# Arktis2022/Spiking-Diffusion

Hardware: AMD Instinct MI355X
Metric: images/sec + LIF-kernel HBM GB/s, MNIST 100-step sample T=16, 1->8 GPU (higher is better)
Workload: dtype fp32-exact (4 fp6 digits x fp4 spikes on the block-scaled MFMA + certified decisions + exact 6-digit recomputation of flagged neurons)

## Files before the change

spiking-diffusion_amd/csrc/den_mfma_fp6v2.hip:

```cpp
#include "den_common.h"
#include "../../include/spkdiff.h"
#include <math.h>
#include <stdlib.h>
#include <type_traits>
#include <utility>

namespace {

typedef int v6i __attribute__((ext_vector_type(6)));
typedef int v8i __attribute__((ext_vector_type(8)));
typedef float v16f __attribute__((ext_vector_type(16)));

constexpr int T16 = 16;
constexpr int CK = 32;
constexpr int POSB = T16 * CK / 2;
constexpr int WT = 64 * 24;
constexpr int N_PAIR = 18;
constexpr int N_D4 = 5;
constexpr int N_MAIN = N_PAIR + N_D4;
constexpr int N_L5 = 2;
constexpr int NACC = 2;
constexpr int W_PIECES = (N_PAIR * WT + 1023) / 1024;
constexpr int W_LDS = W_PIECES * 1024;
constexpr int W_SLAB = ((N_MAIN + N_L5) * WT + 1023) / 1024 * 1024;

constexpr unsigned FLAG_CAP = 1u << 20;

struct V2Args {
  const uint8_t* in0; int nch;
  const uint8_t* wq; const double* scale; const double* bias; const float* wl1;
  const float* bn_a; const float* bn_b;
  uint8_t* out; uint8_t* out_cnt;
  unsigned* flags;
  unsigned flag_cap;
  long long ticket_idx;
  int handover;
  const int* qtab;
  const int* n_dyn;
  const uint8_t* need; const int* cls_cnt; const int* cls_list;
  int B, Cout, Cin;
  int gx, nsets;
};

#define SPK_FP6_PRE "s_nop 1\n\t"
#define SPK_MFMA2(CLS, acc, av, bv, sa, sb)                                                                          \
  asm volatile(SPK_FP6_PRE "v_mfma_scale_f32_32x32x64_f8f6f4 %0, %1, %2, %0, %3, %4 op_sel_hi:[0,0,0] cbsz:4 blgp:2"  \
               : "+" CLS(acc) : "v"(av), "v"(bv), "v"(sa), "v"(sb))
#define SPK_MFMA2_Z(CLS, acc, av, bv, sa, sb)                                                                        \
  asm volatile(SPK_FP6_PRE "v_mfma_scale_f32_32x32x64_f8f6f4 %0, %1, %2, 0, %3, %4 op_sel_hi:[0,0,0] cbsz:4 blgp:2"   \
               : "=&" CLS(acc) : "v"(av), "v"(bv), "v"(sa), "v"(sb))

constexpr int SPK_V2_KMIN = 2;
constexpr float SPK_V2_SPARE = 1.0f;
constexpr int SPK_V2_REC_STEP = 13;
constexpr int SPK_V2_LP_PAIRS = 1;
constexpr int SPK_V2_GX_KB = 2560;
constexpr int SPK_V2_HALF_FILL = 2;
constexpr int SPK_V2_LPS_MIN_B = 64;
constexpr int SPK_V2_LP_SPLIT_MAX = 512;
constexpr int SPK_V2_PF = 6;

constexpr float CERT_4EPS = 4.0f * 2.38418579e-07f;

__device__ __forceinline__ void store_tile_spikes(uint8_t* out, uint8_t* out_cnt, unsigned mybits, int lane, long long rec_base,
                                                  long long cnt_base, bool ok) {
  const unsigned bitsv = spk_transpose16_rows(mybits, lane);
  if (out_cnt && ok) out_cnt[cnt_base + (lane & 31)] = (uint8_t)__popc(mybits);
  if (ok) *reinterpret_cast<uint2*>(out + rec_base + (lane & 15) * 16 + 8 * ((lane >> 4) & 1)) = spk_e2m1_record(bitsv);
}

__device__ const uint8_t V2_HALF_REC[2][64] = {
    {0, 1, 2, 3, 4, 5, 6, 7, 8, 9, 10, 11, 12, 13, 14, 15, 16, 17, 18, 19, 20, 21, 22, 23,
     23, 23, 23, 23, 23, 23, 23, 23, 23, 23, 23, 23, 23, 23, 23, 23, 23, 23, 23, 23, 23, 23, 23, 23, 24},
    {24, 25, 26, 27, 28, 29, 30, 31, 32, 33, 34, 35, 36, 37, 38, 39, 40, 41, 42, 43, 44, 45, 46, 47,
     47, 47, 47, 47, 47, 47, 47, 47, 47, 47, 47, 47, 47, 47, 47, 47, 47, 47, 47, 47, 47, 47, 47, 47, 24}};

template <int H, int W, int NWV, bool SPLIT, int NTP, bool HALF = false>
__device__ __forceinline__ void fp6v2_body(const V2Args& a, const int g, const int il, const int lanes, const int n_images,
                                           const int* __restrict__ slots) {
  constexpr bool PRUNE = NTP > 0;
  static_assert(!HALF || (PRUNE && !SPLIT && H == 7 && W == 7 && NWV == 4 && NTP == 3), "half-image items: 7x7, four waves x three tiles");
  constexpr bool REC = !PRUNE;
  constexpr int HW = H * W, PW = W + 1;
  constexpr int Hb = SPLIT ? H / 2 : H;
  constexpr int Hin = SPLIT ? Hb + 1 : H;
  constexpr int HWb = Hb * W;
  static_assert(SPLIT ? ((H % 2) == 0 && (HWb % (2 * NWV)) == 0)
                      : ((HW & 1) == 1 && ((HW / 2) % NWV) == 0), "whole 32-row tiles on every wave (+ one odd position)");
  static_assert(!PRUNE || (!SPLIT && (NWV == 4 || NWV == 8) && NTP <= (HWb / 2) / NWV), "position lists: 7x7 items");
  constexpr int NT = PRUNE ? NTP : (HWb / 2) / NWV;
  constexpr int N_AGPR = NWV == 4 ? (NACC * NT < 16 ? NACC * NT : 16) : 0;
  constexpr int NPP = (Hin + 2) * PW + 1;
  constexpr int A_BYTES = NPP * POSB;
  constexpr int PPR = (W + 3) / 4;
  constexpr int NA = Hin * PPR;
  constexpr int NPA = (NA + NWV - 1) / NWV;
  constexpr int NPW = (W_PIECES + NWV - 1) / NWV;
  constexpr int NSTEP = 9 * NT;
  static_assert(NWV >= 8 || NACC * NT <= 16 || (NT - 1) * NACC <= N_AGPR + 2, "only the last tile may straddle the register files");
  constexpr bool AH = NWV == 8 && !PRUNE;
  constexpr int NBUF = 2;
  extern __shared__ __attribute__((aligned(16))) uint8_t lds[];
  uint8_t* const sA = lds;
  uint8_t* const sW = lds + NBUF * A_BYTES;
  int* const s_cin = reinterpret_cast<int*>(lds + NBUF * A_BYTES + NBUF * W_LDS);
  int* const s_row = s_cin + NPP * 16;
  int* const s_nmax = s_row + (HWb + 1) * 16;
  const unsigned sA_addr = spk_lds_addr(sA), sW_addr = sA_addr + NBUF * A_BYTES;
  const int tid = threadIdx.x, lane = tid & 63, wave = tid >> 6;
  const int nch = a.nch;
  const int G = a.Cout >> 5;
  for (int i = tid; i < NBUF * A_BYTES / 16; i += NWV * 64) reinterpret_cast<uint4*>(sA)[i] = make_uint4(0, 0, 0, 0);
  if (REC)
    for (int i = tid; i < NPP * 16; i += NWV * 64) s_cin[i] = 0;
  __syncthreads();

  const int row = lane & 31, half = lane >> 5;
  const int hsel = (row >> 2) & 1, tt = (row & 3) + 4 * (row >> 3);
  int a_off[NT];
  int p_out[NT];
#pragma unroll
  for (int i = 0; i < NT; ++i) {
    const int p = 2 * (wave + NWV * i) + hsel;
    a_off[i] = ((p / W) * PW + (p % W)) * POSB + tt * 16;
    p_out[i] = 2 * (wave + NWV * i) + half;
  }

  const int wave_s = __builtin_amdgcn_readfirstlane(wave);
  unsigned pa_pk[NPA];
#pragma unroll
  for (int j = 0; j < NPA; ++j) {
    int id = wave_s * NPA + j;
    id = id < NA ? id : NA - 1;
    const int y = id / PPR, px = id - y * PPR;
    const int np = (W - 4 * px) < 4 ? (W - 4 * px) : 4;
    const unsigned src = (unsigned)((y * W + 4 * px) * POSB), dst = (unsigned)(((y + 1) * PW + 1 + 4 * px) * POSB);
    pa_pk[j] = src | (dst << 14) | ((unsigned)(np - 1) << 29);
  }
  const unsigned lane16 = (unsigned)lane * 16u;
  const unsigned wave_k = (unsigned)wave_s * 1024u;
  auto issue_piece = [&](int q, const uint8_t* aslab, const uint8_t* wslab, unsigned dA, unsigned dW) {
    if (q < NPA) {
      const unsigned pk = pa_pk[q];
      const unsigned np = ((pk >> 29) & 3u) + 1u;
      const unsigned long long mask = np == 4 ? ~0ull : ((1ull << (16 * np)) - 1ull);
      spk_dma16s_masked(aslab + (pk & 0x3fffu), lane16, dA + ((pk >> 14) & 0x7fffu), mask);
    } else {
      unsigned ko = wave_k + 1024u * NWV * (unsigned)(q - NPA);
      if (NWV * (q - NPA) + NWV - 1 >= W_PIECES) ko = ko < (unsigned)W_PIECES * 1024u ? ko : ko - 1024u * NWV;
      spk_dma16s(wslab + ko, lane16, dW + ko);
    }
  };
  const uint8_t* const wbase = a.wq + (long long)g * nch * W_SLAB;
  auto aslab_of = [&](int itm, int c) -> const uint8_t* {
    const int b = HALF ? itm >> 1 : (PRUNE ? slots[itm] : (SPLIT ? itm >> 1 : itm)), band = SPLIT ? itm & 1 : 0;
    return a.in0 + ((long long)b * nch + c) * HW * POSB + band * (Hb - 1) * W * POSB;
  };
  const int nitems = (SPLIT || HALF) ? 2 * n_images : n_images;

  const int co = g * 32 + (lane & 31);
  const float scale_f = (float)a.scale[co], bias_f = (float)a.bias[co];
  const float bna = a.bn_a[co], bnb = a.bn_b[co];
  const float Bc = fmaf(bias_f, bna, bnb);
  const float cE = 2.0f * 2.38418579e-07f * (fabsf(bnb) + fabsf(Bc)) + 1e-30f;
  const float cT = 528.0f * scale_f * fabsf(bna) * 1.000001f;
  const float Ac4 = 1024.0f * scale_f * bna;

  const int sc_a = 0x7f7f7f7f;
  const int sc_p = half ? (int)0x82828282u : (int)0x87878787u;

  int it = 0;
  if (il < nitems) {
    const uint8_t* as0 = aslab_of(il, 0);
#pragma unroll
    for (int q = 0; q < NPA + NPW; ++q) issue_piece(q, as0, wbase, sA_addr, sW_addr);
    if constexpr (AH) {
      spk_dma_wait_all();
      __syncthreads();
    }
  }
  for (int itm = il; itm < nitems; itm += lanes) {
    const int b = HALF ? itm >> 1 : (PRUNE ? slots[itm] : (SPLIT ? itm >> 1 : itm)), band = SPLIT ? itm & 1 : 0;
    const int band_off = band * PW * POSB;
    int n_list = 2 * NT * NWV;
    if constexpr (PRUNE) {
      const uint8_t* rec = HALF ? &V2_HALF_REC[itm & 1][0] : a.need + (long long)b * 64;
      n_list = __builtin_amdgcn_readfirstlane((int)rec[48]);
#pragma unroll
      for (int i = 0; i < NT; ++i) {
        const int k2 = 2 * (wave + NWV * i);
        const int p = rec[k2 + hsel];
        a_off[i] = ((p / W) * PW + (p % W)) * POSB + tt * 16;
        p_out[i] = rec[k2 + half];
      }
    }
    v16f acc[NT][NACC];
    int cnt[NT];
#pragma unroll
    for (int i = 0; i < NT; ++i) cnt[i] = 0;
    constexpr int NREC = Hin * W * 16, NR = (NREC + NWV * 64 - 1) / (NWV * 64);
    int creg[NR];
    int rec_off[NR];
    bool rec_ok[NR];
#pragma unroll
    for (int k = 0; k < NR; ++k) {
      creg[k] = 0;
      const int r = tid + k * NWV * 64;
      const int cl = r >> 4, t = r & 15;
      rec_ok[k] = r < NREC;
      rec_off[k] = rec_ok[k] ? (((cl / W) + 1) * PW + 1 + (cl % W)) * POSB + t * 16 : 0;
    }
    constexpr int PFX = NWV == 4 ? SPK_V2_PF : 4;
    v6i bp[2][2];
    v4i af[PFX];
    for (int c = 0; c < nch; ++c, ++it) {
      const int buf = it & 1, buf1 = buf ^ 1;
      if constexpr (!AH) {
        spk_dma_wait_all();
        __syncthreads();
      }
      int nb = itm, nc = c + 1;
      if (nc == nch) { nc = 0; nb = itm + lanes; }
      const bool have_next = nb < nitems;
      const uint8_t* n_aslab = aslab_of(have_next ? nb : itm, have_next ? nc : c);
      const uint8_t* n_wslab = wbase + (long long)(have_next ? nc : c) * W_SLAB;
      const unsigned n_dA = sA_addr + buf1 * A_BYTES;
      const unsigned n_dW = sW_addr + buf1 * W_LDS;

      v4i rvq[NR];
      auto compute = [&](auto first_tag) {
        constexpr bool FIRST = decltype(first_tag)::value;
        const uint8_t* A = sA + buf * A_BYTES + band_off;
        const uint8_t* Wb = sW + buf * W_LDS;
        auto toff = [](int tap) constexpr -> int { return ((tap / 3) * PW + (tap % 3)) * POSB; };
        constexpr int NBLK = 9;
        auto lda = [&](auto s_tag) -> v4i {
          constexpr int s = decltype(s_tag)::value;
          constexpr int blk = s / NT, i = s % NT;
          return *reinterpret_cast<const v4i*>(A + a_off[i] + toff(blk));
        };
        auto ldb = [&](int tile) -> v6i {
          const uint8_t* p = Wb + tile * WT;
          const v4i x = *reinterpret_cast<const v4i*>(p + lane * 16);
          typedef const volatile __attribute__((address_space(3))) v2i* lds_v2i_ptr;
          const v2i y = *(lds_v2i_ptr)SPK_LDS(p + 1024 + lane * 8);
          const v6i r = {x[0], x[1], x[2], x[3], y[0], y[1]};
          return r;
        };
        constexpr int PF = PFX;
        if constexpr (!AH || FIRST) {
          bp[0][0] = ldb(0); bp[0][1] = ldb(1);
          static_for<PF>([&](auto s_tag) { af[decltype(s_tag)::value] = lda(s_tag); });
        }
        const uint8_t* An = sA + buf1 * A_BYTES + band_off;
        const uint8_t* Wn = sW + buf1 * W_LDS;
        const bool ahead = AH && c + 1 < nch;
        static_for<NSTEP>([&](auto s_tag) {
          constexpr int s = decltype(s_tag)::value;
          constexpr int blk = s / NT, i = s % NT;
          if constexpr (AH && s == NSTEP - PF) {
            asm volatile("s_waitcnt vmcnt(0)\n\ts_barrier" ::: "memory");
          }
          const v4i av = af[s % PF];
          if constexpr (s + PF < NSTEP) af[s % PF] = lda(std::integral_constant<int, s + PF>{});
          else if constexpr (AH) {
            constexpr int k = s % PF;
            if (ahead) af[k] = *reinterpret_cast<const v4i*>(An + a_off[k % NT] + toff(k / NT));
          }
          constexpr int NPIECES = NPA + NPW;
#define V2_DMA_SLOT()                                                                              \
  do {                                                                                             \
    if constexpr (i == 0 && 2 * blk < NPIECES) issue_piece(2 * blk, n_aslab, n_wslab, n_dA, n_dW);     \
    if constexpr (i == (NT > 1 ? NT / 2 : 0) && 2 * blk + 1 < NPIECES)                             \
      issue_piece(2 * blk + 1, n_aslab, n_wslab, n_dA, n_dW);                                      \
  } while (0)
#define V2_NEXT_TILES()                                                                            \
  do {                                                                                             \
    if constexpr (i == 0 && blk + 1 < NBLK) {                                                      \
      bp[(blk + 1) & 1][0] = ldb(2 * (blk + 1));                                                   \
      bp[(blk + 1) & 1][1] = ldb(2 * (blk + 1) + 1);                                               \
    }                                                                                              \
  } while (0)
          constexpr int tap = blk;
          if constexpr (!REC) {
            asm volatile("v_bcnt_u32_b32 %0, %1, %0\n\tv_bcnt_u32_b32 %0, %2, %0\n\tv_bcnt_u32_b32 %0, %3, %0\n\t"
                         "v_bcnt_u32_b32 %0, %4, %0" : "+v"(cnt[i]) : "v"(av[0]), "v"(av[1]), "v"(av[2]), "v"(av[3]));
          }
#define V2_PAIR_MFMA(J)                                                                                      \
do {                                                                                                        \
  if constexpr (FIRST && tap == 0) {                                                                        \
    if constexpr (NACC * i + (J) < N_AGPR) SPK_MFMA2_Z("a", acc[i][J], av, bp[0][J], sc_a, sc_p);              \
    else SPK_MFMA2_Z("v", acc[i][J], av, bp[0][J], sc_a, sc_p);                                             \
  } else {                                                                                                  \
    if constexpr (NACC * i + (J) < N_AGPR) SPK_MFMA2("a", acc[i][J], av, bp[tap & 1][J], sc_a, sc_p);          \
    else SPK_MFMA2("v", acc[i][J], av, bp[tap & 1][J], sc_a, sc_p);                                         \
  }                                                                                                         \
} while (0)
          V2_PAIR_MFMA(0);
          __builtin_amdgcn_sched_barrier(0);
          V2_DMA_SLOT();
          V2_NEXT_TILES();
          if constexpr (REC) {
            if constexpr (s == 1) {
#pragma unroll
              for (int k = 0; k < NR; ++k) rvq[k] = *reinterpret_cast<const v4i*>(sA + buf * A_BYTES + rec_off[k]);
            }
            if constexpr (s == SPK_V2_REC_STEP) {
#pragma unroll
              for (int k = 0; k < NR; ++k)
                creg[k] += __builtin_popcount((unsigned)rvq[k][0]) + __builtin_popcount((unsigned)rvq[k][1]) +
                           __builtin_popcount((unsigned)rvq[k][2]) + __builtin_popcount((unsigned)rvq[k][3]);
            }
          }
          V2_PAIR_MFMA(1);
          __builtin_amdgcn_sched_barrier(0);
          if constexpr (AH && s == NSTEP - 1) {
            if (ahead) {
              auto ldb_n = [&](int tile) -> v6i {
                const uint8_t* p = Wn + tile * WT;
                const v4i x = *reinterpret_cast<const v4i*>(p + lane * 16);
                typedef const volatile __attribute__((address_space(3))) v2i* lds_v2i_ptr;
                const v2i y = *(lds_v2i_ptr)SPK_LDS(p + 1024 + lane * 8);
                const v6i r = {x[0], x[1], x[2], x[3], y[0], y[1]};
                return r;
              };
              bp[0][0] = ldb_n(0); bp[0][1] = ldb_n(1);
            }
          }
        });
      };
      if (c == 0) compute(std::true_type{}); else compute(std::false_type{});
    }

    if constexpr (REC) {
#pragma unroll
      for (int k = 0; k < NR; ++k)
        if (rec_ok[k]) s_cin[(rec_off[k] / POSB) * 16 + ((rec_off[k] % POSB) >> 4)] = creg[k];
      if (tid <= HWb) s_nmax[tid] = 0;
      __syncthreads();
      for (int e = tid; e < HWb * 16; e += NWV * 64) {
        const int pp = e >> 4, t = e & 15;
        const int* c0 = s_cin + (((pp / W) + band) * PW + (pp % W)) * 16 + t;
        int sum = 0;
#pragma unroll
        for (int dy = 0; dy < 3; ++dy)
#pragma unroll
          for (int dx = 0; dx < 3; ++dx) sum += c0[(dy * PW + dx) * 16];
        s_row[e] = sum;
        atomicMax(&s_nmax[pp], sum);
      }
      __syncthreads();
    }
    asm volatile("s_nop 15\n\ts_nop 15" ::: "memory");

#pragma unroll
    for (int k = 0; k < NT; ++k) {
      const int i = k == 0 ? NT - 1 : k - 1;
#pragma unroll
      for (int j = 0; j < NACC; ++j)
        if (NACC * i + j < N_AGPR) asm volatile("" : "+a"(acc[i][j]));
      float v = 0.f;
      unsigned mybits = 0;
      bool flg = false;
      int cntv[16];
      if constexpr (!REC) {
#pragma unroll
        for (int r = 0; r < 16; ++r) {
          const int rowA = (r & 3) + 8 * (r >> 2);
          const int c0 = __builtin_amdgcn_readlane(cnt[i], rowA), c1 = __builtin_amdgcn_readlane(cnt[i], rowA + 4);
          cntv[r] = half ? c1 : c0;
        }
      }
      int nmax_rec = 0;
      if constexpr (REC) nmax_rec = s_nmax[2 * (wave + NWV * i) + half];
      typedef float v2f __attribute__((ext_vector_type(2)));
      float zmax = 0.f, dmin = 3.0e38f;
      int nmax = nmax_rec;
#pragma unroll
      for (int r2 = 0; r2 < 16; r2 += 2) {
        const v2f p0 = {acc[i][0][r2], acc[i][0][r2 + 1]}, p1 = {acc[i][1][r2], acc[i][1][r2 + 1]};
        const v2f q4 = __builtin_elementwise_fma(p0, (v2f){1024.0f, 1024.0f}, p1);
        const v2f z2 = __builtin_elementwise_fma(q4, (v2f){Ac4, Ac4}, (v2f){Bc, Bc});
        if constexpr (!REC) nmax = max(nmax, max(cntv[r2], cntv[r2 + 1]));
#pragma unroll
        for (int e = 0; e < 2; ++e) {
          const float z = z2[e];
          zmax = fmaxf(zmax, fabsf(z));
          const float h = fmaf(z - v, 0.5f, v);
          const float hm = h - 1.0f;
          dmin = fminf(dmin, fabsf(hm));
          const bool s = h >= 1.0f;
          v = s ? 0.0f : h;
          mybits = __builtin_amdgcn_alignbit(mybits, __float_as_uint(hm), 31);
        }
      }
      mybits = ~(__builtin_bitreverse32(mybits) >> 16) & 0xffffu;
      flg = dmin <= SPK_V2_SPARE * fmaf(zmax, 2.5f * CERT_4EPS, fmaf((float)nmax, cT, cE));
      if (__builtin_amdgcn_ballot_w64(flg) != 0ull) {
        float v2 = 0.f, dh = 0.f;
        bool f2 = false;
        if constexpr (REC) {
          const v4i* rp = reinterpret_cast<const v4i*>(s_row + (2 * (wave + NWV * i) + half) * 16);
#pragma unroll
          for (int q = 0; q < 4; ++q) {
            const v4i c4 = rp[q];
            cntv[4 * q] = c4[0]; cntv[4 * q + 1] = c4[1]; cntv[4 * q + 2] = c4[2]; cntv[4 * q + 3] = c4[3];
          }
        }
#pragma unroll
        for (int r2 = 0; r2 < 16; r2 += 2) {
          const v2f p0 = {acc[i][0][r2], acc[i][0][r2 + 1]}, p1 = {acc[i][1][r2], acc[i][1][r2 + 1]};
          const v2f q4 = __builtin_elementwise_fma(p0, (v2f){1024.0f, 1024.0f}, p1);
          const v2f z2 = __builtin_elementwise_fma(q4, (v2f){Ac4, Ac4}, (v2f){Bc, Bc});
#pragma unroll
          for (int e = 0; e < 2; ++e) {
            const float z = z2[e];
            const float ct = fmaf((float)cntv[r2 + e], cT, cE);
            dh = fmaf(fabsf(z) + fabsf(v2), 0.625f * CERT_4EPS, fmaf(dh, 0.5f, 0.5f * ct));
            const float h = fmaf(z - v2, 0.5f, v2);
            f2 = f2 || (fabsf(h - 1.0f) <= SPK_V2_SPARE * dh);
            v2 = h >= 1.0f ? 0.0f : h;
          }
        }
        flg = flg && f2;
      }
      const int ti = wave + NWV * i;
      const int p = PRUNE ? p_out[i] : 2 * ti + half + band * HWb;
      const bool listed = !PRUNE || 2 * ti + half < n_list;
      if (flg && listed) {
        const long long n = ((long long)b * a.Cout + co) * HW + p;
        const unsigned idx = atomicAdd(a.flags, 1u);
        if (idx < a.flag_cap) a.flags[2 + idx] = (unsigned)n;
        else atomicOr(a.flags + 2 + FLAG_CAP + (n >> 5), 1u << (n & 31));
      }
      const long long rec = (((long long)b * G + g) * HW + p) * POSB;
      store_tile_spikes(a.out, a.out_cnt, mybits, lane, rec, (((long long)b * G + g) * HW + p) * 32, listed);
      __builtin_amdgcn_sched_barrier(0);
    }
  }
  spk_dma_wait_all();
}

__device__ __forceinline__ void fp6v2_wg_map(const V2Args& a, int& g, int& il, int& lanes) {
  const int k = blockIdx.x, G = a.Cout >> 5;
  if (a.gx > 0) {
    const int S = gridDim.x >> 3, x = k & 7, slot = k >> 3;
    const int npart = 8 / a.nsets, set = x % a.nsets, xi = x / a.nsets, lanes_x = S / a.gx;
    g = set * a.gx + slot % a.gx;
    il = xi * lanes_x + slot / a.gx;
    lanes = npart * lanes_x;
  } else {
    g = k % G;
    il = k / G;
    lanes = gridDim.x / G;
  }
}

__device__ __forceinline__ void fp6v2_handover(const V2Args& a) {
  if (!a.handover) return;
  __syncthreads();
  if (threadIdx.x == 0) {
    if (atomicAdd(a.flags + a.ticket_idx, 1u) == gridDim.x - 1) {
      a.flags[1] = atomicAdd(a.flags, 0u);
      a.flags[0] = 0u;
      a.flags[a.ticket_idx] = 0u;
    }
  }
}


template <int H, int W, int NWV, bool SPLIT = false>
__global__ __launch_bounds__(NWV * 64, 1) void conv3x3_fp6v2_kernel(V2Args a) {
  const int Bn = a.n_dyn ? (*a.n_dyn < a.B ? *a.n_dyn : a.B) : a.B;
  int g, il, lanes;
  fp6v2_wg_map(a, g, il, lanes);
  fp6v2_body<H, W, NWV, SPLIT, 0>(a, g, il, lanes, Bn, nullptr);
  fp6v2_handover(a);
}

template <int H, int W>
__global__ __launch_bounds__(256, 1) void conv3x3_fp6v2_half_kernel(V2Args a) {
  const int Bn = a.n_dyn ? (*a.n_dyn < a.B ? *a.n_dyn : a.B) : a.B;
  int g, il, lanes;
  fp6v2_wg_map(a, g, il, lanes);
  fp6v2_body<H, W, 4, false, 3, true>(a, g, il, lanes, Bn, nullptr);
  fp6v2_handover(a);
}

template <int H, int W, int NWV>
__global__ __launch_bounds__(NWV * 64, 1) void conv3x3_fp6v2_listed_kernel(V2Args a) {
  constexpr int NC = (H * W / 2) / 4;
  int g, il, lanes;
  fp6v2_wg_map(a, g, il, lanes);
  int cnt[NC], work[NC], u[NC];
  int total = 0, nonempty = 0;
#pragma unroll
  for (int k = 0; k < NC; ++k) {
    cnt[k] = a.cls_cnt[k];
    work[k] = cnt[k] * (k + 1 < SPK_V2_KMIN ? SPK_V2_KMIN : k + 1);
    total += work[k];
    nonempty += cnt[k] > 0;
  }
  if (total == 0) { fp6v2_handover(a); return; }
  int rem = lanes - nonempty, used = 0;
#pragma unroll
  for (int k = 0; k < NC; ++k) {
    u[k] = cnt[k] > 0 ? 1 + (int)((long long)rem * work[k] / total) : 0;
    used += u[k];
  }
  for (int left = lanes - used; left > 0; --left) {
    int best = 0;
    long long bw = -1, bu = 1;
#pragma unroll
    for (int k = 0; k < NC; ++k)
      if (cnt[k] > 0 && (long long)work[k] * bu > bw * u[k]) { bw = work[k]; bu = u[k]; best = k; }
#pragma unroll
    for (int k = 0; k < NC; ++k) u[k] += (k == best);
  }
  int start = 0, cls = -1, il_c = 0, lanes_c = 1;
#pragma unroll
  for (int k = 0; k < NC; ++k) {
    if (il >= start && il < start + u[k]) { cls = k; il_c = il - start; lanes_c = u[k]; }
    start += u[k];
  }
  const int* slots = a.cls_list + (long long)(cls < 0 ? 0 : cls) * a.B;
  static_assert(NWV == 8, "listed positions: two waves per SIMD");
  switch (cls) {
    case 0: case 1: fp6v2_body<H, W, 8, false, 1>(a, g, il_c, lanes_c, cnt[cls], slots); break;
    case 2: case 3: fp6v2_body<H, W, 8, false, 2>(a, g, il_c, lanes_c, cnt[cls], slots); break;
    case 4: case 5: fp6v2_body<H, W, 8, false, 3>(a, g, il_c, lanes_c, cnt[cls], slots); break;
    default: break;
  }
  fp6v2_handover(a);
}

__device__ __forceinline__ float exact_preact(double s, double sc, double bi) { return (float)fma(s, sc, bi); }

template <int H, int W, bool WIDE>
__device__ __forceinline__ void fp6v2_lastpos_body(const V2Args& a, const int bid, float (*red)[16][64]) {
  constexpr int HW = H * W, NP = SPK_V2_LP_PAIRS;
  const int lane = threadIdx.x & 63, wave = threadIdx.x >> 6;
  const int nch = a.nch, G = a.Cout >> 5;
  const int Bn = a.n_dyn ? (*a.n_dyn < a.B ? *a.n_dyn : a.B) : a.B;
  if (!a.handover && bid == 0 && threadIdx.x == 0) { a.flags[1] = a.flags[0]; a.flags[0] = 0u; }
  const int n_units = ((Bn + 2 * NP - 1) / (2 * NP)) * G;
  const bool split = n_units <= SPK_V2_LP_SPLIT_MAX;
  const int unit = split ? bid : bid * 4 + wave;
  const int g = unit % G, b0 = (unit / G) * 2 * NP;
  if (b0 >= Bn) return;
  const int row = lane & 31, half = lane >> 5;
  const int hsel = (row >> 2) & 1, tt = (row & 3) + 4 * (row >> 3);
  const int sc_a = 0x7f7f7f7f;
  const int sc_p = half ? (int)0x82828282u : (int)0x87878787u;
  const int sc_hi = (int)0x87878787u, sc_lo = (int)0x82828282u;
  v16f acc[NP][3];
#pragma unroll
  for (int q = 0; q < NP; ++q)
#pragma unroll
    for (int j = 0; j < 3; ++j)
#pragma unroll
      for (int r = 0; r < 16; ++r) acc[q][j][r] = 0.f;
  const int py = H - 1, px = W - 1;
  for (int c = split ? wave : 0; c < nch; c += split ? 4 : 1) {
    const uint8_t* wslab = a.wq + ((long long)g * nch + c) * W_SLAB;
    auto ldb = [&](int tile) -> v8i {
      const uint8_t* wt = wslab + tile * WT;
      const v4i bx = *reinterpret_cast<const v4i*>(wt + lane * 16);
      const v2i by = *reinterpret_cast<const v2i*>(wt + 1024 + lane * 8);
      return v8i{bx[0], bx[1], bx[2], bx[3], by[0], by[1], 0, 0};
    };
    v4i sp[NP][4];
#pragma unroll
    for (int q = 0; q < NP; ++q) {
      const int bA = b0 + 2 * q + hsel;
#pragma unroll
      for (int u = 0; u < 4; ++u) {
        const int tap = (u >> 1) * 3 + (u & 1);
        const int yy = py + tap / 3 - 1, xx = px + tap % 3 - 1;
        sp[q][u] = v4i{0, 0, 0, 0};
        if (bA < Bn)
          sp[q][u] = *reinterpret_cast<const v4i*>(a.in0 + (((long long)bA * nch + c) * HW + yy * W + xx) * POSB + tt * 16);
      }
    }
    v8i bt[8];
#pragma unroll
    for (int u = 0; u < 4; ++u) {
      const int tap = (u >> 1) * 3 + (u & 1);
      bt[2 * u] = ldb(2 * tap); bt[2 * u + 1] = ldb(2 * tap + 1);
    }
    const v8i t18 = ldb(N_PAIR), t19 = ldb(N_PAIR + 1), t20 = ldb(N_PAIR + 2), t23 = ldb(N_MAIN), t24 = ldb(N_MAIN + 1);
    auto mm = [&](v16f& d, const v4i& av, const v8i& bv, int sb) {
      const v8i a8 = {av[0], av[1], av[2], av[3], 0, 0, 0, 0};
      d = __builtin_amdgcn_mfma_scale_f32_32x32x64_f8f6f4(a8, bv, d, 4, 2, 0, sc_a, 0, sb);
    };
    const v4i zero = {0, 0, 0, 0};
#pragma unroll
    for (int q = 0; q < NP; ++q) {
#pragma unroll
      for (int u = 0; u < 4; ++u) { mm(acc[q][0], sp[q][u], bt[2 * u], sc_p); mm(acc[q][1], sp[q][u], bt[2 * u + 1], sc_p); }
      const v4i a01 = half ? sp[q][1] : sp[q][0];
      const v4i az3 = half ? sp[q][2] : zero;
      const v4i a4z = half ? zero : sp[q][3];
      const v4i a34 = half ? sp[q][3] : sp[q][2];
      mm(acc[q][2], a01, t18, sc_hi); mm(acc[q][2], az3, t19, sc_hi); mm(acc[q][2], a4z, t20, sc_hi);
      mm(acc[q][2], a01, t23, sc_lo); mm(acc[q][2], a34, t24, sc_lo);
    }
  }
  if (split) {
    const int nw = nch < 4 ? nch : 4;
    if constexpr (WIDE) {
#pragma unroll
      for (int q = 0; q < NP; ++q) {
        if (q) __syncthreads();
        if (wave != 0 && wave < nw) {
#pragma unroll
          for (int j = 0; j < 3; ++j)
#pragma unroll
            for (int r = 0; r < 16; ++r) red[3 * (wave - 1) + j][r][lane] = acc[q][j][r];
        }
        __syncthreads();
        if (wave == 0) {
          for (int w = 1; w < nw; ++w)
#pragma unroll
            for (int j = 0; j < 3; ++j)
#pragma unroll
              for (int r = 0; r < 16; ++r) acc[q][j][r] += red[3 * (w - 1) + j][r][lane];
        }
      }
    } else {
#pragma unroll
      for (int q = 0; q < NP; ++q)
        for (int w = 1; w < 4; ++w) {
          if (wave == w && w < nw) {
#pragma unroll
            for (int j = 0; j < 3; ++j)
#pragma unroll
              for (int r = 0; r < 16; ++r) red[j][r][lane] = acc[q][j][r];
          }
          __syncthreads();
          if (wave == 0 && w < nw) {
#pragma unroll
            for (int j = 0; j < 3; ++j)
#pragma unroll
              for (int r = 0; r < 16; ++r) acc[q][j][r] += red[j][r][lane];
          }
          __syncthreads();
        }
    }
    if (wave != 0) return;
  }
  const int co = g * 32 + (lane & 31);
  const double sc = a.scale[co], bi = a.bias[co];
  const float bna = a.bn_a[co], bnb = a.bn_b[co];
#pragma unroll
  for (int q = 0; q < NP; ++q) {
    const int b = b0 + 2 * q + half;
    const bool ok = b < Bn;
    if (__builtin_amdgcn_ballot_w64(ok) == 0ull) continue;
    float v = 0.f;
    unsigned mybits = 0;
#pragma unroll
    for (int r = 0; r < 16; ++r) {
      const double s1 = fma((double)acc[q][0][r], 1024.0, (double)acc[q][1][r]);
      const double s = fma(s1, 1024.0, (double)acc[q][2][r]);
      const float y = exact_preact(s, sc, bi);
      const bool sp1 = spk_lif_step_default(v, fmaf(y, bna, bnb)) && ok;
      mybits |= sp1 ? (1u << r) : 0u;
    }
    const long long cell = ((long long)(ok ? b : 0) * G + g) * HW + (HW - 1);
    store_tile_spikes(a.out, a.out_cnt, mybits, lane, cell * POSB, cell * 32, ok);
  }
}

template <int H, int W>
__device__ __forceinline__ void fixup_neuron(const V2Args& a, long long n, unsigned long long* sS, int Bn) {
  constexpr int HW = H * W;
  const int tid = threadIdx.x, lane = tid & 63;
  const int nch = a.nch, Cin = a.Cin;
  const int p = (int)(n % HW);
  const long long r0 = n / HW;
  const int co = (int)(r0 % a.Cout), b = (int)(r0 / a.Cout);
  if (b >= Bn) return;
  const int py = p / W, px = p % W;
  if (tid < 16) sS[tid] = 0ull;
  long long part = 0;
  __syncthreads();
  const int units = 9 * nch * 16;
  for (int u = tid; u < units; u += (int)blockDim.x) {
    const int t = u & 15, cc = (u >> 4) % nch, tap = (u >> 4) / nch;
    const int yy = py + tap / 3 - 1, xx = px + tap % 3 - 1;
    if (yy < 0 || yy >= H || xx < 0 || xx >= W) continue;
    const uint4 sp = *reinterpret_cast<const uint4*>(a.in0 + (((long long)b * nch + cc) * HW + yy * W + xx) * POSB + t * 16);
    const int4* qp = reinterpret_cast<const int4*>(a.qtab + ((long long)co * 9 + tap) * Cin + cc * 32);
    const unsigned w4[4] = {sp.x, sp.y, sp.z, sp.w};
#pragma unroll
    for (int j = 0; j < 8; ++j) {
      const int4 q = qp[j];
      const unsigned nib = w4[j >> 1] >> (16 * (j & 1));
      part += (nib & 0x000fu) ? (long long)q.x : 0ll;
      part += (nib & 0x00f0u) ? (long long)q.y : 0ll;
      part += (nib & 0x0f00u) ? (long long)q.z : 0ll;
      part += (nib & 0xf000u) ? (long long)q.w : 0ll;
    }
  }
#pragma unroll
  for (int off = 16; off <= 32; off <<= 1) {
    const int lo = __shfl_xor((int)(unsigned)(part & 0xffffffffll), off);
    const int hi = __shfl_xor((int)(part >> 32), off);
    part += (long long)(((unsigned long long)(unsigned)hi << 32) | (unsigned)lo);
  }
  if (lane < 16 && part != 0) atomicAdd(&sS[lane], (unsigned long long)part);
  __syncthreads();
  if (tid < 64) {
    const double sc = a.scale[co], bi = a.bias[co];
    const float bna = a.bn_a[co], bnb = a.bn_b[co];
    float v = 0.f;
    unsigned bits = 0;
#pragma unroll
    for (int t = 0; t < 16; ++t) {
      const float y = exact_preact((double)(long long)sS[t], sc, bi);
      bits |= spk_lif_step_default(v, fmaf(y, bna, bnb)) ? (1u << t) : 0u;
    }
    const int g = co >> 5;
    if (lane < 16) {
      uint8_t* rec = a.out + ((((long long)b * (a.Cout >> 5) + g) * HW + p) * POSB);
      const int byte = (co & 31) >> 1;
      const unsigned shw = 8u * (byte & 3) + 4u * (co & 1);
      unsigned* wp = reinterpret_cast<unsigned*>(rec + lane * 16 + (byte & ~3));
      atomicAnd(wp, ~(0xFu << shw));
      if ((bits >> lane) & 1u) atomicOr(wp, 0x2u << shw);
    }
    if (a.out_cnt && lane == 0) a.out_cnt[(((long long)b * (a.Cout >> 5) + g) * HW + p) * 32 + (co & 31)] = (uint8_t)__popc(bits);
  }
  __syncthreads();
}

template <int H, int W>
__device__ __forceinline__ void fp6v2_fixup_body(const V2Args& a, long long n_words, const unsigned bid, const unsigned nb,
                                                 unsigned long long* sS) {
  const int Bn = a.n_dyn ? (*a.n_dyn < a.B ? *a.n_dyn : a.B) : a.B;
  const unsigned count = a.flags[a.handover ? 1 : 0];
  const unsigned nlist = count < a.flag_cap ? count : a.flag_cap;
  for (unsigned e = bid; e < nlist; e += nb) fixup_neuron<H, W>(a, (long long)a.flags[2 + e], sS, Bn);
  if (count > a.flag_cap) {
    unsigned* bm = a.flags + 2 + FLAG_CAP;
    const long long per = (n_words + nb - 1) / nb;
    const long long w0 = (long long)bid * per;
    const long long w1 = w0 + per < n_words ? w0 + per : n_words;
    for (long long wi = w0; wi < w1; ++wi) {
      unsigned wv = bm[wi];
      __syncthreads();
      if (threadIdx.x == 0 && wv) bm[wi] = 0u;
      while (wv) {
        const int bit = __ffs((int)wv) - 1;
        wv &= wv - 1;
        fixup_neuron<H, W>(a, wi * 32 + bit, sS, Bn);
      }
    }
  }
}

constexpr int LPS_TILES = 13, LPS_BUF = LPS_TILES * WT;
constexpr size_t LPS_LDS = 2 * (size_t)LPS_BUF;
template <int H, int W>
__device__ __forceinline__ void fp6v2_lastpos_shared_body(const V2Args& a, const int bid) {
  constexpr int HW = H * W;
  extern __shared__ __attribute__((aligned(16))) uint8_t lds[];
  const int lane = threadIdx.x & 63, wave = threadIdx.x >> 6;
  const int nch = a.nch, G = a.Cout >> 5;
  const int Bn = a.n_dyn ? (*a.n_dyn < a.B ? *a.n_dyn : a.B) : a.B;
  const int g = bid % G, b0 = (bid / G) * 8;
  if (b0 >= Bn) return;
  const int row = lane & 31, half = lane >> 5;
  const int hsel = (row >> 2) & 1, tt = (row & 3) + 4 * (row >> 3);
  const int sc_a = 0x7f7f7f7f;
  const int sc_p = half ? (int)0x82828282u : (int)0x87878787u;
  const int sc_hi = (int)0x87878787u, sc_lo = (int)0x82828282u;
  const int wave_s = __builtin_amdgcn_readfirstlane(wave);
  const unsigned lds_addr = spk_lds_addr(lds), lane16 = (unsigned)lane * 16u;
// ... 356 lines not shown
```

Before: 2811.

## Skip zero-padding taps for border waves in full 7x7 fp6 conv items

Reassigns output positions on 8-wave full 7x7 items so that four waves hold only top, left, right or bottom border positions, and gives each wave class a compile-time tap plan that omits the 3x3 taps that fall entirely in zero padding. Each class is instantiated as a separate template body selected per wave, so those waves issue fewer MFMA steps and weight-tile loads. The DMA slot and weight prefetch schedule are re-indexed by block within the plan. Interior waves still do all nine taps, so whole-workgroup time may be bound by them, and the extra template instances increase code size.

Measured after the change: 3098, median of 6. 1.1x the previous value.

```diff
diff --git a/spiking-diffusion_amd/csrc/den_mfma_fp6v2.hip b/spiking-diffusion_amd/csrc/den_mfma_fp6v2.hip
--- a/spiking-diffusion_amd/csrc/den_mfma_fp6v2.hip
+++ b/spiking-diffusion_amd/csrc/den_mfma_fp6v2.hip
@@ -75,7 +75,61 @@
     {24, 25, 26, 27, 28, 29, 30, 31, 32, 33, 34, 35, 36, 37, 38, 39, 40, 41, 42, 43, 44, 45, 46, 47,
      47, 47, 47, 47, 47, 47, 47, 47, 47, 47, 47, 47, 47, 47, 47, 47, 47, 47, 47, 47, 47, 47, 47, 47, 24}};
 
-template <int H, int W, int NWV, bool SPLIT, int NTP, bool HALF = false>
+enum : int { V2_INT = 0, V2_TOP, V2_RIGHT, V2_LEFT, V2_BOTTOM, V2_NCLS };
+struct V2Plan { int nblk; int tap[9]; int nt[9]; };
+constexpr int V2_FT = 3;
+constexpr V2Plan V2_PLAN[V2_NCLS] = {
+    {9, {0, 1, 2, 3, 4, 5, 6, 7, 8}, {3, 3, 3, 3, 3, 3, 3, 3, 3}},
+    {6, {3, 4, 5, 6, 7, 8}, {3, 3, 3, 3, 3, 3}},
+    {6, {0, 1, 3, 4, 6, 7}, {3, 3, 3, 3, 3, 3}},
+    {6, {1, 2, 4, 5, 7, 8}, {3, 3, 3, 3, 3, 3}},
+    {9, {0, 6, 7, 8, 1, 2, 3, 4, 5}, {3, 1, 1, 1, 3, 3, 3, 3, 3}}};
+constexpr V2Plan v2_uniform_plan(int nt) {
+  V2Plan p = {9, {0, 1, 2, 3, 4, 5, 6, 7, 8}, {}};
+  for (int b = 0; b < 9; ++b) p.nt[b] = nt;
+  return p;
+}
+constexpr int v2_plan_start(const V2Plan& p, int blk) {
+  int n = 0;
+  for (int b = 0; b < blk; ++b) n += p.nt[b];
+  return n;
+}
+constexpr int v2_plan_blk(const V2Plan& p, int s) {
+  int b = 0;
+  while (s >= p.nt[b]) s -= p.nt[b++];
+  return b;
+}
+__device__ constexpr uint8_t V2_FULL_POS[8][V2_FT][2] = {
+    {{0, 1}, {2, 3}, {4, 5}},       {{6, 13}, {20, 27}, {34, 41}},  {{7, 14}, {21, 28}, {35, 42}},  {{43, 44}, {45, 46}, {47, 40}},
+    {{8, 9}, {10, 11}, {12, 15}},   {{16, 17}, {18, 19}, {22, 23}}, {{24, 25}, {26, 29}, {30, 31}}, {{32, 33}, {36, 37}, {38, 39}}};
+__device__ constexpr uint8_t V2_WAVE_CLS[8] = {V2_TOP, V2_RIGHT, V2_LEFT, V2_BOTTOM, V2_INT, V2_INT, V2_INT, V2_INT};
+constexpr bool v2_full_map_ok() {
+  bool seen[48] = {};
+  for (int w = 0; w < 8; ++w)
+    for (int i = 0; i < V2_FT; ++i)
+      for (int h = 0; h < 2; ++h) {
+        const int p = V2_FULL_POS[w][i][h];
+        if (p >= 48 || seen[p]) return false;
+        seen[p] = true;
+      }
+  for (int w = 0; w < 8; ++w) {
+    const V2Plan& pl = V2_PLAN[V2_WAVE_CLS[w]];
+    for (int i = 0; i < V2_FT; ++i)
+      for (int tap = 0; tap < 9; ++tap) {
+        int n = 0;
+        for (int b = 0; b < pl.nblk; ++b) n += pl.tap[b] == tap && i >= V2_FT - pl.nt[b];
+        if (n > 1) return false;
+        for (int h = 0; h < 2 && n == 0; ++h) {
+          const int y = V2_FULL_POS[w][i][h] / 7 + tap / 3 - 1, x = V2_FULL_POS[w][i][h] % 7 + tap % 3 - 1;
+          if (y >= 0 && y < 7 && x >= 0 && x < 7) return false;
+        }
+      }
+  }
+  return true;
+}
+static_assert(v2_full_map_ok(), "full 7x7 items: position table and block lists");
+
+template <int H, int W, int NWV, bool SPLIT, int NTP, bool HALF = false, int CLS = V2_INT>
 __device__ __forceinline__ void fp6v2_body(const V2Args& a, const int g, const int il, const int lanes, const int n_images,
                                            const int* __restrict__ slots) {
   constexpr bool PRUNE = NTP > 0;
@@ -96,7 +150,9 @@
   constexpr int NA = Hin * PPR;
   constexpr int NPA = (NA + NWV - 1) / NWV;
   constexpr int NPW = (W_PIECES + NWV - 1) / NWV;
-  constexpr int NSTEP = 9 * NT;
+  constexpr bool BSKIP = NWV == 8 && !PRUNE && !SPLIT;
+  static_assert(!BSKIP || (H == 7 && W == 7 && NT == V2_FT), "border skip: the position table is for 7x7 items of three tiles per wave");
+  static_assert(BSKIP || CLS == V2_INT, "wave classes: full 7x7 items only");
   static_assert(NWV >= 8 || NACC * NT <= 16 || (NT - 1) * NACC <= N_AGPR + 2, "only the last tile may straddle the register files");
   constexpr bool AH = NWV == 8 && !PRUNE;
   constexpr int NBUF = 2;
@@ -121,9 +177,9 @@
   int p_out[NT];
 #pragma unroll
   for (int i = 0; i < NT; ++i) {
-    const int p = 2 * (wave + NWV * i) + hsel;
+    const int p = BSKIP ? (int)V2_FULL_POS[wave & 7][i % V2_FT][hsel] : 2 * (wave + NWV * i) + hsel;
     a_off[i] = ((p / W) * PW + (p % W)) * POSB + tt * 16;
-    p_out[i] = 2 * (wave + NWV * i) + half;
+    p_out[i] = BSKIP ? (int)V2_FULL_POS[wave & 7][i % V2_FT][half] : 2 * (wave + NWV * i) + half;
   }
 
   const int wave_s = __builtin_amdgcn_readfirstlane(wave);
@@ -233,12 +289,21 @@
         const uint8_t* A = sA + buf * A_BYTES + band_off;
         const uint8_t* Wb = sW + buf * W_LDS;
         auto toff = [](int tap) constexpr -> int { return ((tap / 3) * PW + (tap % 3)) * POSB; };
-        constexpr int NBLK = 9;
-        auto lda = [&](auto s_tag) -> v4i {
+        constexpr V2Plan P = BSKIP ? V2_PLAN[CLS] : v2_uniform_plan(NT);
+        constexpr int NBLK = P.nblk, NSTEP = v2_plan_start(P, NBLK);
+        constexpr int PF = PFX;
+        constexpr int NPIECES = NPA + NPW;
+        static_assert(P.nt[0] == NT, "the first block writes (not accumulates) every accumulator");
+        static_assert(2 * NBLK >= NPIECES, "two copy slots per block: every DMA piece of the wave gets one");
+        static_assert((!AH || NSTEP >= 2 * PF) && (!REC || NSTEP > SPK_V2_REC_STEP), "look-ahead slots; the record-count steps exist");
+        static_assert(!AH || (v2_plan_start(P, (NPIECES + 1) / 2) <= NSTEP - PF && v2_plan_start(P, NBLK - 2) <= NSTEP - PF),
+                      "chunk barrier behind the copies and the last weight-tile read");
+        auto lda_at = [&](const uint8_t* base, auto s_tag) -> v4i {
           constexpr int s = decltype(s_tag)::value;
-          constexpr int blk = s / NT, i = s % NT;
-          return *reinterpret_cast<const v4i*>(A + a_off[i] + toff(blk));
+          constexpr int blk = v2_plan_blk(P, s), i = NT - P.nt[blk] + (s - v2_plan_start(P, blk));
+          return *reinterpret_cast<const v4i*>(base + a_off[i] + toff(P.tap[blk]));
         };
+        auto lda = [&](auto s_tag) -> v4i { return lda_at(A, s_tag); };
         auto ldb = [&](int tile) -> v6i {
           const uint8_t* p = Wb + tile * WT;
           const v4i x = *reinterpret_cast<const v4i*>(p + lane * 16);
@@ -247,9 +312,8 @@
           const v6i r = {x[0], x[1], x[2], x[3], y[0], y[1]};
           return r;
         };
-        constexpr int PF = PFX;
         if constexpr (!AH || FIRST) {
-          bp[0][0] = ldb(0); bp[0][1] = ldb(1);
+          bp[0][0] = ldb(2 * P.tap[0]); bp[0][1] = ldb(2 * P.tap[0] + 1);
           static_for<PF>([&](auto s_tag) { af[decltype(s_tag)::value] = lda(s_tag); });
         }
         const uint8_t* An = sA + buf1 * A_BYTES + band_off;
@@ -257,7 +321,8 @@
         const bool ahead = AH && c + 1 < nch;
         static_for<NSTEP>([&](auto s_tag) {
           constexpr int s = decltype(s_tag)::value;
-          constexpr int blk = s / NT, i = s % NT;
+          constexpr int blk = v2_plan_blk(P, s), nt = P.nt[blk], j = s - v2_plan_start(P, blk);
+          constexpr int i = NT - nt + j;
           if constexpr (AH && s == NSTEP - PF) {
             asm volatile("s_waitcnt vmcnt(0)\n\ts_barrier" ::: "memory");
           }
@@ -265,35 +330,33 @@
           if constexpr (s + PF < NSTEP) af[s % PF] = lda(std::integral_constant<int, s + PF>{});
           else if constexpr (AH) {
             constexpr int k = s % PF;
-            if (ahead) af[k] = *reinterpret_cast<const v4i*>(An + a_off[k % NT] + toff(k / NT));
+            if (ahead) af[k] = lda_at(An, std::integral_constant<int, k>{});
           }
-          constexpr int NPIECES = NPA + NPW;
 #define V2_DMA_SLOT()                                                                              \
   do {                                                                                             \
-    if constexpr (i == 0 && 2 * blk < NPIECES) issue_piece(2 * blk, n_aslab, n_wslab, n_dA, n_dW);     \
-    if constexpr (i == (NT > 1 ? NT / 2 : 0) && 2 * blk + 1 < NPIECES)                             \
+    if constexpr (j == 0 && 2 * blk < NPIECES) issue_piece(2 * blk, n_aslab, n_wslab, n_dA, n_dW);     \
+    if constexpr (j == (nt > 1 ? nt / 2 : 0) && 2 * blk + 1 < NPIECES)                             \
       issue_piece(2 * blk + 1, n_aslab, n_wslab, n_dA, n_dW);                                      \
   } while (0)
 #define V2_NEXT_TILES()                                                                            \
   do {                                                                                             \
-    if constexpr (i == 0 && blk + 1 < NBLK) {                                                      \
-      bp[(blk + 1) & 1][0] = ldb(2 * (blk + 1));                                                   \
-      bp[(blk + 1) & 1][1] = ldb(2 * (blk + 1) + 1);                                               \
+    if constexpr (j == 0 && blk + 1 < NBLK) {                                                      \
+      bp[(blk + 1) & 1][0] = ldb(2 * P.tap[(blk + 1) % 9]);                                        \
+      bp[(blk + 1) & 1][1] = ldb(2 * P.tap[(blk + 1) % 9] + 1);                                    \
     }                                                                                              \
   } while (0)
-          constexpr int tap = blk;
           if constexpr (!REC) {
             asm volatile("v_bcnt_u32_b32 %0, %1, %0\n\tv_bcnt_u32_b32 %0, %2, %0\n\tv_bcnt_u32_b32 %0, %3, %0\n\t"
                          "v_bcnt_u32_b32 %0, %4, %0" : "+v"(cnt[i]) : "v"(av[0]), "v"(av[1]), "v"(av[2]), "v"(av[3]));
           }
 #define V2_PAIR_MFMA(J)                                                                                      \
 do {                                                                                                        \
-  if constexpr (FIRST && tap == 0) {                                                                        \
+  if constexpr (FIRST && blk == 0) {                                                                        \
     if constexpr (NACC * i + (J) < N_AGPR) SPK_MFMA2_Z("a", acc[i][J], av, bp[0][J], sc_a, sc_p);              \
     else SPK_MFMA2_Z("v", acc[i][J], av, bp[0][J], sc_a, sc_p);                                             \
   } else {                                                                                                  \
-    if constexpr (NACC * i + (J) < N_AGPR) SPK_MFMA2("a", acc[i][J], av, bp[tap & 1][J], sc_a, sc_p);          \
-    else SPK_MFMA2("v", acc[i][J], av, bp[tap & 1][J], sc_a, sc_p);                                         \
+    if constexpr (NACC * i + (J) < N_AGPR) SPK_MFMA2("a", acc[i][J], av, bp[blk & 1][J], sc_a, sc_p);          \
+    else SPK_MFMA2("v", acc[i][J], av, bp[blk & 1][J], sc_a, sc_p);                                         \
   }                                                                                                         \
 } while (0)
           V2_PAIR_MFMA(0);
@@ -324,7 +387,7 @@
                 const v6i r = {x[0], x[1], x[2], x[3], y[0], y[1]};
                 return r;
               };
-              bp[0][0] = ldb_n(0); bp[0][1] = ldb_n(1);
+              bp[0][0] = ldb_n(2 * P.tap[0]); bp[0][1] = ldb_n(2 * P.tap[0] + 1);
             }
           }
         });
@@ -372,7 +435,7 @@
         }
       }
       int nmax_rec = 0;
-      if constexpr (REC) nmax_rec = s_nmax[2 * (wave + NWV * i) + half];
+      if constexpr (REC) nmax_rec = s_nmax[BSKIP ? p_out[i] : 2 * (wave + NWV * i) + half];
       typedef float v2f __attribute__((ext_vector_type(2)));
       float zmax = 0.f, dmin = 3.0e38f;
       int nmax = nmax_rec;
@@ -400,7 +463,7 @@
         float v2 = 0.f, dh = 0.f;
         bool f2 = false;
         if constexpr (REC) {
-          const v4i* rp = reinterpret_cast<const v4i*>(s_row + (2 * (wave + NWV * i) + half) * 16);
+          const v4i* rp = reinterpret_cast<const v4i*>(s_row + (BSKIP ? p_out[i] : 2 * (wave + NWV * i) + half) * 16);
 #pragma unroll
           for (int q = 0; q < 4; ++q) {
             const v4i c4 = rp[q];
@@ -425,7 +488,7 @@
         flg = flg && f2;
       }
       const int ti = wave + NWV * i;
-      const int p = PRUNE ? p_out[i] : 2 * ti + half + band * HWb;
+      const int p = (PRUNE || BSKIP) ? p_out[i] : 2 * ti + half + band * HWb;
       const bool listed = !PRUNE || 2 * ti + half < n_list;
       if (flg && listed) {
         const long long n = ((long long)b * a.Cout + co) * HW + p;
@@ -474,7 +537,15 @@
   const int Bn = a.n_dyn ? (*a.n_dyn < a.B ? *a.n_dyn : a.B) : a.B;
   int g, il, lanes;
   fp6v2_wg_map(a, g, il, lanes);
-  fp6v2_body<H, W, NWV, SPLIT, 0>(a, g, il, lanes, Bn, nullptr);
+  if constexpr (NWV == 8 && !SPLIT) {
+    switch (__builtin_amdgcn_readfirstlane((int)V2_WAVE_CLS[(threadIdx.x >> 6) & 7])) {
+      case V2_TOP: fp6v2_body<H, W, NWV, false, 0, false, V2_TOP>(a, g, il, lanes, Bn, nullptr); break;
+      case V2_RIGHT: fp6v2_body<H, W, NWV, false, 0, false, V2_RIGHT>(a, g, il, lanes, Bn, nullptr); break;
+      case V2_LEFT: fp6v2_body<H, W, NWV, false, 0, false, V2_LEFT>(a, g, il, lanes, Bn, nullptr); break;
+      case V2_BOTTOM: fp6v2_body<H, W, NWV, false, 0, false, V2_BOTTOM>(a, g, il, lanes, Bn, nullptr); break;
+      default: fp6v2_body<H, W, NWV, false, 0, false, V2_INT>(a, g, il, lanes, Bn, nullptr); break;
+    }
+  } else fp6v2_body<H, W, NWV, SPLIT, 0>(a, g, il, lanes, Bn, nullptr);
   fp6v2_handover(a);
 }
 
```
